# simeonjunker/retr

Measured on AMD Instinct MI355X. Metric: RefCOCO images/sec (train fwd+bwd) at 1/2/4/8 GPUs; greedy-decode refs/sec, higher is better.
Workload: dtype bf16; 1 GPU; cfg2: ResNet-50 + 6-enc/6-dec d_model 256, 640x640, batch 16/GPU, fwd+CE+bwd+allreduce+clip+AdamW; global_batch=16, seq_len=128, parallelism=dp1

## Files before the change

### retr_amd/csrc/conv.hip

```cpp
#include <algorithm>
#include <cstring>
#include <vector>

#include "gemm2.hpp"
#include "panel.hpp"
#include "epilogues.hpp"
#include "../../include/retr_hip.h"

using namespace retr;

namespace retr {
bool conv3x3_direct_ok(int H, int W, int CI, int CO);
int conv3x3_fwd_direct(const bf16* x, const bf16* w, const float* bias, bf16* y, int relu, int Nb,
                       int H, int W, int CI, int CO, hipStream_t st);
int conv3x3_dgrad_direct(const bf16* dy, const bf16* wt, bf16* dx, const bf16* addend,
                         const bf16* gate, int Nb, int H, int W, int CI_out, int CO_in,
                         hipStream_t st);
}

namespace {

struct Geom {
  int Nb, H, W, C, Co, KH, KW, s, p, d, OH, OW;
};

struct TapCur {
  int k, c, kw, khd, kwd;
};
RETR_DEVICE TapCur tap_cur(int k, int Cc, int KW, int dil) {
  TapCur t;
  t.k = k;
  int khw = k / Cc;
  t.c = k - khw * Cc;
  int kh = khw / KW;
  t.kw = khw - kh * KW;
  t.khd = kh * dil;
  t.kwd = t.kw * dil;
  return t;
}
RETR_DEVICE void tap_advance(TapCur& t, int d, int Cc, int KW, int dil) {
  t.k += d;
  t.c += d;
  while (t.c >= Cc) {
    t.c -= Cc;
    if (++t.kw == KW) {
      t.kw = 0;
      t.kwd = 0;
      t.khd += dil;
    } else {
      t.kwd += dil;
    }
  }
}

template <typename T>
struct ConvFwdA {
  static constexpr bool kContig = true;
  const T* x;
  Geom g;
  int M, K;
  struct Ctx { const T* img; int ihb, iwb; bool ok; };
  using KCur = TapCur;
  RETR_DEVICE Ctx row_ctx(int r) const {
    Ctx c;
    c.ok = r < M;
    int rr = c.ok ? r : 0;
    int hw = g.OH * g.OW;
    int n = rr / hw, rem = rr - n * hw;
    int oh = rem / g.OW, ow = rem - oh * g.OW;
    c.img = x + (long)n * g.H * g.W * g.C;
    c.ihb = oh * g.s - g.p;
    c.iwb = ow * g.s - g.p;
    return c;
  }
  RETR_DEVICE KCur kcur(int k) const { return tap_cur(k, g.C, g.KW, g.d); }
  RETR_DEVICE void advance(KCur& t, int d) const { tap_advance(t, d, g.C, g.KW, g.d); }
  RETR_DEVICE const void* addr(const Ctx& c, const KCur& t) const {
    if (!c.ok || t.k >= K) return nullptr;
    int ih = c.ihb + t.khd, iw = c.iwb + t.kwd;
    if ((unsigned)ih >= (unsigned)g.H || (unsigned)iw >= (unsigned)g.W) return nullptr;
    return c.img + ((long)ih * g.W + iw) * g.C + t.c;
  }
};

template <typename T>
struct ConvFwdAU {
  static constexpr bool kContig = true;
  static constexpr bool kUniformK = true;
  const T* x;
  Geom g;
  int M, K;
  struct Ctx { const T* base; unsigned mask; };
  struct KCur { int c0, t, kh, kw, off; };
  RETR_DEVICE Ctx row_ctx_c(int r, int coff) const {
    Ctx c;
    const bool ok = r < M;
    const int rr = ok ? r : 0;
    const int hw = g.OH * g.OW;
    const int n = rr / hw, rem = rr - n * hw;
    const int oh = rem / g.OW, ow = rem - oh * g.OW;
    const int ihb = oh * g.s - g.p, iwb = ow * g.s - g.p;
    c.base = x + (((long)n * g.H + ihb) * g.W + iwb) * g.C + coff;
    unsigned m = 0;
    if (ok) {
      for (int kh = 0; kh < g.KH; ++kh)
        for (int kw = 0; kw < g.KW; ++kw)
          if ((unsigned)(ihb + kh * g.d) < (unsigned)g.H &&
              (unsigned)(iwb + kw * g.d) < (unsigned)g.W)
            m |= 1u << (kh * g.KW + kw);
    }
    c.mask = m;
    return c;
  }
  RETR_DEVICE Ctx row_ctx(int r) const { return row_ctx_c(r, 0); }
  RETR_DEVICE void set_off(KCur& t) const { t.off = (t.kh * g.d * g.W + t.kw * g.d) * g.C + t.c0; }
  RETR_DEVICE KCur kcur(int k) const {
    KCur t;
    t.t = k / g.C;
    t.c0 = k - t.t * g.C;
    t.kh = t.t / g.KW;
    t.kw = t.t - t.kh * g.KW;
    set_off(t);
    return t;
  }
  RETR_DEVICE void advance(KCur& t, int d) const {
    t.c0 += d;
    if (t.c0 >= g.C) {
      t.c0 -= g.C;
      ++t.t;
      if (++t.kw == g.KW) {
        t.kw = 0;
        ++t.kh;
      }
    }
    set_off(t);
  }
  RETR_DEVICE const void* addr(const Ctx& c, const KCur& t) const {
    if (!((c.mask >> t.t) & 1u)) return nullptr;
    return c.base + t.off;
  }
  RETR_DEVICE const void* addr_or(const Ctx& c, const KCur& t, const void* fb) const {
    return ((c.mask >> t.t) & 1u) ? (const void*)(c.base + t.off) : fb;
  }
};

template <typename T>
struct ConvDgradA {
  static constexpr bool kContig = true;
  const T* gr;
  Geom g;
  int M, K;
  struct Ctx { const T* img; int ihp, iwp; bool ok; };
  using KCur = TapCur;
  RETR_DEVICE Ctx row_ctx(int r) const {
    Ctx c;
    c.ok = r < M;
    int rr = c.ok ? r : 0;
    int hw = g.H * g.W;
    int n = rr / hw, rem = rr - n * hw;
    int ih = rem / g.W, iw = rem - ih * g.W;
    c.img = gr + (long)n * g.OH * g.OW * g.Co;
    c.ihp = ih + g.p;
    c.iwp = iw + g.p;
    return c;
  }
  RETR_DEVICE KCur kcur(int k) const { return tap_cur(k, g.Co, g.KW, g.d); }
  RETR_DEVICE void advance(KCur& t, int d) const { tap_advance(t, d, g.Co, g.KW, g.d); }
  RETR_DEVICE const void* addr(const Ctx& c, const KCur& t) const {
    if (!c.ok || t.k >= K) return nullptr;
    int th = c.ihp - t.khd, tw = c.iwp - t.kwd;
    if (th < 0 || tw < 0) return nullptr;
    int oh = th, ow = tw;
    if (g.s != 1) {
      oh = th / g.s;
      ow = tw / g.s;
      if (oh * g.s != th || ow * g.s != tw) return nullptr;
    }
    if (oh >= g.OH || ow >= g.OW) return nullptr;
    return c.img + ((long)oh * g.OW + ow) * g.Co + t.c;
  }
};

template <typename T>
struct ConvDgradAU {
  static constexpr bool kContig = true;
  static constexpr bool kUniformK = true;
  const T* gr;
  Geom g;
  int M, K;
  struct Ctx { const T* base; unsigned mask; };
  struct KCur { int c0, t, kh, kw, off; };
  RETR_DEVICE Ctx row_ctx_c(int r, int coff) const {
    Ctx c;
    const bool ok = r < M;
    const int rr = ok ? r : 0;
    const int hw = g.H * g.W;
    const int n = rr / hw, rem = rr - n * hw;
    const int ih = rem / g.W, iw = rem - ih * g.W;
    const int ihp = ih + g.p, iwp = iw + g.p;
    c.base = gr + (((long)n * g.OH + ihp) * g.OW + iwp) * g.Co + coff;
    unsigned m = 0;
    if (ok) {
      for (int kh = 0; kh < g.KH; ++kh)
        for (int kw = 0; kw < g.KW; ++kw)
          if ((unsigned)(ihp - kh * g.d) < (unsigned)g.OH &&
              (unsigned)(iwp - kw * g.d) < (unsigned)g.OW)
            m |= 1u << (kh * g.KW + kw);
    }
    c.mask = m;
    return c;
  }
  RETR_DEVICE Ctx row_ctx(int r) const { return row_ctx_c(r, 0); }
  RETR_DEVICE void set_off(KCur& t) const {
    t.off = t.c0 - (t.kh * g.d * g.OW + t.kw * g.d) * g.Co;
  }
  RETR_DEVICE KCur kcur(int k) const {
    KCur t;
    t.t = k / g.Co;
    t.c0 = k - t.t * g.Co;
    t.kh = t.t / g.KW;
    t.kw = t.t - t.kh * g.KW;
    set_off(t);
    return t;
  }
  RETR_DEVICE void advance(KCur& t, int d) const {
    t.c0 += d;
    if (t.c0 >= g.Co) {
      t.c0 -= g.Co;
      ++t.t;
      if (++t.kw == g.KW) {
        t.kw = 0;
        ++t.kh;
      }
    }
    set_off(t);
  }
  RETR_DEVICE const void* addr(const Ctx& c, const KCur& t) const {
    if (!((c.mask >> t.t) & 1u)) return nullptr;
    return c.base + t.off;
  }
  RETR_DEVICE const void* addr_or(const Ctx& c, const KCur& t, const void* fb) const {
    return ((c.mask >> t.t) & 1u) ? (const void*)(c.base + t.off) : fb;
  }
};

template <typename T>
struct ConvWgradB {
  static constexpr bool kContig = false;
  const T* x;
  Geom g;
  int rows, M;
  int adv_q, adv_r;
  struct Ctx { int khd, kwd; long off; bool ok; };
  struct KCur { int m, oh, ow; long base; };
  RETR_DEVICE Ctx row_ctx(int r) const {
    Ctx c;
    c.ok = r < rows;
    int rr = c.ok ? r : 0;
    int khw = rr / g.C;
    const int ci = rr - khw * g.C;
    int kh = khw / g.KW, kw = khw - kh * g.KW;
    c.khd = kh * g.d - g.p;
    c.kwd = kw * g.d - g.p;
    c.off = ((long)c.khd * g.W + c.kwd) * g.C + ci;
    return c;
  }
  RETR_DEVICE KCur kcur(int m) const {
    KCur k;
    k.m = m;
    int hw = g.OH * g.OW;
    const int n = m / hw;
    int rem = m - n * hw;
    k.oh = rem / g.OW;
    k.ow = rem - k.oh * g.OW;
    k.base = (((long)n * g.H + k.oh * g.s) * g.W + k.ow * g.s) * g.C;
    return k;
  }
  RETR_DEVICE void advance(KCur& k, int d) const {
    k.m += d;
    if (d != Elem<T>::BK) {
      k = kcur(k.m);
      return;
    }
    const long rowC = (long)g.s * g.W * g.C;
    k.ow += adv_r;
    k.oh += adv_q;
    k.base += (long)adv_q * rowC + (long)adv_r * g.s * g.C;
    if (k.ow >= g.OW) {
      k.ow -= g.OW;
      k.oh += 1;
      k.base += rowC - (long)g.OW * g.s * g.C;
    }
    while (k.oh >= g.OH) {
      k.oh -= g.OH;
      k.base += ((long)g.H - (long)g.OH * g.s) * g.W * g.C;
    }
  }
  RETR_DEVICE const void* addr(const Ctx& c, const KCur& k) const {
    if (!c.ok || k.m >= M) return nullptr;
    int ih = k.oh * g.s + c.khd, iw = k.ow * g.s + c.kwd;
    if ((unsigned)ih >= (unsigned)g.H || (unsigned)iw >= (unsigned)g.W) return nullptr;
    return x + k.base + c.off;
  }
};

template <typename T>
struct ConvWgradB32 {
  static constexpr bool kContig = false;
  const T* x;
  Geom g;
  int rows, M;
  int adv_q, adv_r;
  int d_step, d_row, d_img;
  struct Ctx { int khd, kwd, off; bool ok; };
  struct KCur { int m, oh, ow, base; };
  RETR_DEVICE Ctx row_ctx(int r) const {
    Ctx c;
    c.ok = r < rows;
    const int rr = c.ok ? r : 0;
    const int khw = rr / g.C;
// ... 131 lines not shown
    c.mask = m;
    return c;
  }
  RETR_DEVICE Ctx row_ctx(int r) const { return row_ctx_c(r, 0); }
  RETR_DEVICE void set_off(KCur& t) const { t.off = t.c0 - (t.ti * g.OW + t.tj) * g.Co; }
  RETR_DEVICE KCur kcur(int k) const {
    KCur t;
    t.t = k / g.Co;
    t.c0 = k - t.t * g.Co;
    t.ti = t.t / ph.nkw;
    t.tj = t.t - t.ti * ph.nkw;
    set_off(t);
    return t;
  }
  RETR_DEVICE void advance(KCur& t, int d) const {
    t.c0 += d;
    if (t.c0 >= g.Co) {
      t.c0 -= g.Co;
      ++t.t;
      if (++t.tj == ph.nkw) {
        t.tj = 0;
        ++t.ti;
      }
    }
    set_off(t);
  }
  RETR_DEVICE const void* addr(const Ctx& c, const KCur& t) const {
    if (!((c.mask >> t.t) & 1u)) return nullptr;
    return c.base + t.off;
  }
  RETR_DEVICE const void* addr_or(const Ctx& c, const KCur& t, const void* fb) const {
    return ((c.mask >> t.t) & 1u) ? (const void*)(c.base + t.off) : fb;
  }
};

template <typename T>
struct DgradPhaseWU {
  static constexpr bool kContig = true;
  static constexpr bool kUniformK = true;
  const T* wt;
  Geom g;
  Phase ph;
  int rows, K;
  struct Ctx { const T* row; int klim; };
  struct KCur { int k, c0, ti, tj, off; };
  RETR_DEVICE Ctx row_ctx_c(int r, int coff) const {
    return Ctx{wt + (long)(r < rows ? r : 0) * g.KH * g.KW * g.Co + coff, r < rows ? K : 0};
  }
  RETR_DEVICE Ctx row_ctx(int r) const { return row_ctx_c(r, 0); }
  RETR_DEVICE void set_off(KCur& t) const {
    t.off = ((ph.a + 2 * t.ti) * g.KW + ph.b + 2 * t.tj) * g.Co + t.c0;
  }
  RETR_DEVICE KCur kcur(int k) const {
    KCur t;
    t.k = k;
    const int tap = k / g.Co;
    t.c0 = k - tap * g.Co;
    t.ti = tap / ph.nkw;
    t.tj = tap - t.ti * ph.nkw;
    set_off(t);
    return t;
  }
  RETR_DEVICE void advance(KCur& t, int d) const {
    t.k += d;
    t.c0 += d;
    if (t.c0 >= g.Co) {
      t.c0 -= g.Co;
      if (++t.tj == ph.nkw) {
        t.tj = 0;
        ++t.ti;
      }
    }
    set_off(t);
  }
  RETR_DEVICE const void* addr(const Ctx& c, const KCur& t) const {
    return t.k < c.klim ? (const void*)(c.row + t.off) : nullptr;
  }
  RETR_DEVICE const void* addr_or(const Ctx& c, const KCur& t, const void* fb) const {
    return t.k < c.klim ? (const void*)(c.row + t.off) : fb;
  }
};

template <typename T>
struct DgradPhaseW {
  static constexpr bool kContig = true;
  const T* wt;
  Geom g;
  Phase ph;
  int rows, K;
  struct Ctx { const T* row; bool ok; };
  struct KCur { int k, c, ti, tj; };
  RETR_DEVICE Ctx row_ctx(int r) const {
    return Ctx{wt + (long)(r < rows ? r : 0) * g.KH * g.KW * g.Co, r < rows};
  }
  RETR_DEVICE KCur kcur(int k) const {
    KCur t;
    t.k = k;
    const int tap = k / g.Co;
    t.c = k - tap * g.Co;
    t.ti = tap / ph.nkw;
    t.tj = tap - t.ti * ph.nkw;
    return t;
  }
  RETR_DEVICE void advance(KCur& t, int d) const {
    t.k += d;
    t.c += d;
    while (t.c >= g.Co) {
      t.c -= g.Co;
      if (++t.tj == ph.nkw) {
        t.tj = 0;
        ++t.ti;
      }
    }
  }
  RETR_DEVICE const void* addr(const Ctx& c, const KCur& t) const {
    if (!c.ok || t.k >= K) return nullptr;
    const int kh = ph.a + 2 * t.ti, kw = ph.b + 2 * t.tj;
    return c.row + ((long)kh * g.KW + kw) * g.Co + t.c;
  }
};

template <class EP>
struct EpiPhaseRows {
  EP ep;
  int Hp, Wp, H, W, ih0, iw0;
  static constexpr bool kRowSum = false;
  float* rowsum = nullptr;
  RETR_DEVICE int map(int m) const {
    const int hw = Hp * Wp;
    const int n = m / hw, rem = m - n * hw;
    const int i = rem / Wp, j = rem - i * Wp;
    return (n * H + ih0 + 2 * i) * W + iw0 + 2 * j;
  }
  RETR_DEVICE void apply(int m, int n, float v) const { ep.apply(map(m), n, v); }
  RETR_DEVICE void apply8(int m, int n, float (&v)[8]) const { ep.apply8(map(m), n, v); }
  using Pre = typename EP::Pre;
  RETR_DEVICE void fetch8(int m, int n, Pre& p) const { ep.fetch8(map(m), n, p); }
  RETR_DEVICE void apply8p(int m, int n, float (&v)[8], const Pre& p) const {
    ep.apply8p(map(m), n, v, p);
  }
  RETR_DEVICE void empty_split(int, int) const {}
  RETR_DEVICE bool lane_contiguous() const { return false; }
};

inline bool prefer_tile64(int M, int N, int K, bool dense1x1, bool res_small_k) {
  if (retr_tune_get(RETR_TUNE_BIG_TILE) != 0) return false;
  if (res_small_k) return true;
  if (M <= 8192 && (N <= 512 || K <= 512)) return true;
  return dense1x1 && N >= 1024 && K <= 512 && M <= 32768;
}

template <int FAM, typename T, class LA, class LB, class EP>
int launch_auto(const LA& la, const LB& lb, const EP& ep, int M, int N, int K, int splits,
                hipStream_t st, const char* what, bool dense1x1 = false,
                bool res_small_k = false) {
  if constexpr (sizeof(T) == 2) {
    return launch_big<FAM>(la, lb, ep, M, N, K, splits, st, what,
                           prefer_tile64(M, N, K, dense1x1, res_small_k));
  } else {
    if (N >= 128 && M >= 4096) return launch_gemm<FAM, T, 128, 128>(la, lb, ep, M, N, K, splits, st, what);
    return launch_gemm<FAM, T, 64, 64>(la, lb, ep, M, N, K, splits, st, what);
  }
}

struct WgradPlan {
  int tile;
  int splits;
};

template <typename T>
WgradPlan wgrad_plan(int R, int Ncols, int Mp, bool dense1x1) {
  constexpr int BK = Elem<T>::BK;
  WgradPlan p{64, 1};
  if (R >= 128 && Ncols >= 128) p.tile = sizeof(T) == 2 ? 128 : 129;
  const int tt = retr_tune_get(RETR_TUNE_CONV_WGRAD_TILE);
  if (sizeof(T) == 2 && R >= 64 && Ncols >= 64 &&
      (tt == 1 || (tt == 0 && dense1x1 && (R <= 128 || Ncols <= 128 || Mp <= 8192))))
    p.tile = 65;
  if (p.tile == 65 && tt == 3) p.tile = 66;
  const int bm = (p.tile == 64 || p.tile == 65 || p.tile == 66) ? 64 : 128;
  const int bn = bm;
  const long tiles = (long)cdiv(R, bm) * cdiv(Ncols, bn);
  const int ksteps = cdiv(Mp, BK);
  const int tune = retr_tune_get(RETR_TUNE_CONV_WGRAD_SPLITS);
  long smax = ksteps / 8;
  if (smax > 128) smax = 128;
  if (smax < 1) smax = 1;
  long s;
  if (tune >= 2) {
    s = tune < smax ? tune : smax;
  } else if (tune == 1 || (p.tile != 128 && p.tile != 65 && p.tile != 66)) {
    s = (512 + tiles - 1) / tiles;
    if (s > smax) s = smax;
  } else {
    const long slots = p.tile == 66 ? 2048 : p.tile == 65 ? 1024 : 512;
    const double slab_cost = p.tile == 128 ? 0.016 : 0.004;
    s = 1;
    double best = 1e30;
    for (long c = 1; c <= smax; ++c) {
      const long kc = cdiv(ksteps, (int)c);
      const long rounds = (tiles * cdiv(ksteps, (int)kc) + slots - 1) / slots;
      const double cost = (double)rounds * (kc + 2) + slab_cost * (double)tiles * c;
      if (cost < best) { best = cost; s = c; }
    }
  }
  if (s < 1) s = 1;
  const int kchunk = cdiv(ksteps, (int)s) * BK;
  p.splits = cdiv(Mp, kchunk);
  return p;
}

template <int FAM, typename T, class LA, class LB>
int launch_wgrad(const LA& la, const LB& lb, float* ws, long ldws, int R, int Ncols, int Mp,
                 hipStream_t st, const char* what, bool dense1x1) {
  const WgradPlan p = wgrad_plan<T>(R, Ncols, Mp, dense1x1);
  const int s = p.splits;
  EpiAccF32 ep{ws, ldws, 0, 0, 1, nullptr};
  ep.split_stride = s > 1 ? (long)R * ldws : 0;
  ep.set_vec();
  if constexpr (sizeof(T) == 2) {
    if (p.tile == 128 && !dense1x1)
      return launch_gemm2<FAM, 128, 128, 4, 2, 2>(la, lb, ep, R, Ncols, Mp, s, st, what);
    if (p.tile == 128) return launch_gemm2<FAM, 128, 128, 2, 2, 2>(la, lb, ep, R, Ncols, Mp, s, st, what);
    if (p.tile == 65) return launch_gemm2<FAM, 64, 64, 2, 2, 2>(la, lb, ep, R, Ncols, Mp, s, st, what);
    if (p.tile == 66) return launch_gemm2<FAM, 64, 64, 2, 2, 1>(la, lb, ep, R, Ncols, Mp, s, st, what);
  } else {
    if (p.tile == 129) return launch_gemm<FAM, T, 128, 128>(la, lb, ep, R, Ncols, Mp, s, st, what);
  }
  return launch_gemm<FAM, T, 64, 64>(la, lb, ep, R, Ncols, Mp, s, st, what);
}

template <typename T>
int conv_fwd_t(const void* x, Geom g, const void* w, const float* bias, const void* res, void* y,
               int relu, hipStream_t st) {
  int M = g.Nb * g.OH * g.OW, N = g.Co, K = g.KH * g.KW * g.C;
  DenseK<T> lb{(const T*)w, (long)K, N, K};
  EpiFwd<T, T> ep{(T*)y, (long)N, bias, (const T*)res, (long)N, relu ? 2 : 0, DropoutParams{0, 0, 1.f}, 0};
  ep.set_vec();
  if (g.KH == 1 && g.KW == 1 && g.s == 1 && g.p == 0) {
    DenseK<T> la{(const T*)x, (long)g.C, M, K};
    if constexpr (sizeof(T) == 2) {
      if (K <= 256 && K % 64 == 0 && N >= 1024 && retr_tune_get(RETR_TUNE_PANEL) == 1 &&
          retr_tune_get(RETR_TUNE_PANEL_CONV) == 1)
        return launch_panel<kFamConvFwd>(la, lb, ep, M, N, K, st, "conv_fwd_1x1");
    }
    return launch_auto<kFamConvFwd, T>(la, lb, ep, M, N, K, 1, st, "conv_fwd_1x1", true,
                                       res != nullptr && K <= 64);
  }
  if constexpr (sizeof(T) == 2) {
    if (g.KH == 3 && g.KW == 3 && g.s == 1 && g.p == 1 && g.d == 1 && !res && relu &&
        conv3x3_direct_ok(g.H, g.W, g.C, g.Co))
      return conv3x3_fwd_direct((const bf16*)x, (const bf16*)w, bias, (bf16*)y, relu, g.Nb, g.H,
                                g.W, g.C, g.Co, st);
  }
  if (sizeof(T) == 2 && g.C % 64 == 0 && g.KH * g.KW > 1 && g.KH * g.KW <= 32) {
    ConvFwdAU<T> la{(const T*)x, g, M, K};
    return launch_auto<kFamConvFwd, T>(la, lb, ep, M, N, K, 1, st, "conv_fwd");
  }
  ConvFwdA<T> la{(const T*)x, g, M, K};
  return launch_auto<kFamConvFwd, T>(la, lb, ep, M, N, K, 1, st, "conv_fwd");
}

__global__ void dgrad_phase_fill_kernel(bf16* dx, const bf16* addend, const bf16* gate, int H,
                                        int W, int C, long chunks, int zmask) {
  const long i = blockIdx.x * (long)blockDim.x + threadIdx.x;
  if (i >= chunks) return;
  const int cpp = C / 8;
  const long p = i / cpp;
  const int c = (int)(i - p * cpp) * 8;
  const int iw = (int)(p % W), ih = (int)((p / W) % H);
  if (!((zmask >> ((ih & 1) * 2 + (iw & 1))) & 1)) return;
  const long off = p * C + c;
  bf16x8 v;
  if (addend) {
    v = *(const bf16x8*)(addend + off);
  } else {
#pragma unroll
    for (int e = 0; e < 8; ++e) v[e] = (bf16)0.f;
  }
  if (gate) {
    const bf16x8 gg = *(const bf16x8*)(gate + off);
#pragma unroll
    for (int e = 0; e < 8; ++e)
      if (!((float)gg[e] > 0.f)) v[e] = (bf16)0.f;
  }
  *(bf16x8*)(dx + off) = v;
}

template <typename T>
int conv_dgrad_t(const void* dy, Geom g, const void* wt, void* dx, const void* addend,
                 const void* gate, hipStream_t st) {
  int M = g.Nb * g.H * g.W, N = g.C, K = g.KH * g.KW * g.Co;
  DenseK<T> lb{(const T*)wt, (long)K, N, K};
  EpiDgrad<T, T, T> ep{(T*)dx, (long)N, (const T*)addend, (long)N, (const T*)gate, (long)N};
  ep.set_vec();
  if (g.KH == 1 && g.KW == 1 && g.s == 1 && g.p == 0) {
    DenseK<T> la{(const T*)dy, (long)g.Co, M, K};
    if constexpr (sizeof(T) == 2) {
      if (K <= 256 && K % 64 == 0 && N >= 1024 && retr_tune_get(RETR_TUNE_PANEL) == 1 &&
          retr_tune_get(RETR_TUNE_PANEL_CONV) == 1)
        return launch_panel<kFamConvDgrad>(la, lb, ep, M, N, K, st, "conv_dgrad_1x1");
    }
    return launch_auto<kFamConvDgrad, T>(la, lb, ep, M, N, K, 1, st, "conv_dgrad_1x1", true);
  }
  if (g.s == 2 && g.d == 1) {
    int zmask = 0;
    for (int a = 0; a < 2; ++a)
      for (int bb = 0; bb < 2; ++bb) {
        const int nkh = g.KH > a ? (g.KH - a + 1) / 2 : 0;
        const int nkw = g.KW > bb ? (g.KW - bb + 1) / 2 : 0;
        if (nkh * nkw == 0) {
          const int ih0 = ((a - g.p) % 2 + 2) % 2, iw0 = ((bb - g.p) % 2 + 2) % 2;
          zmask |= 1 << (ih0 * 2 + iw0);
        }
      }
    const bool inplace = addend != nullptr && addend == dx;
    if (zmask && (inplace || (sizeof(T) == 2 && N % 8 == 0))) {
      if (!inplace) {
        const long chunks = (long)M * (N / 8);
        hipLaunchKernelGGL(dgrad_phase_fill_kernel, dim3((unsigned)cdiv(chunks, 256)), dim3(256),
                           0, st, (bf16*)dx, (const bf16*)addend, (const bf16*)gate, g.H, g.W, N,
                           chunks, zmask);
        if (int e = retr_check_launch("conv_dgrad_phase_fill")) return e;
      }
    } else {
      zmask = 0;
    }
    for (int a = 0; a < 2; ++a)
      for (int bb = 0; bb < 2; ++bb) {
        Phase ph;
        ph.a = a;
        ph.b = bb;
        ph.ih0 = ((a - g.p) % 2 + 2) % 2;
        ph.iw0 = ((bb - g.p) % 2 + 2) % 2;
        ph.Hp = g.H > ph.ih0 ? (g.H - ph.ih0 + 1) / 2 : 0;
        ph.Wp = g.W > ph.iw0 ? (g.W - ph.iw0 + 1) / 2 : 0;
        ph.nkh = g.KH > a ? (g.KH - a + 1) / 2 : 0;
        ph.nkw = g.KW > bb ? (g.KW - bb + 1) / 2 : 0;
        const int Mp = g.Nb * ph.Hp * ph.Wp, Kp = ph.nkh * ph.nkw * g.Co;
        if (Mp == 0) continue;
        if (Kp == 0 && (zmask >> (ph.ih0 * 2 + ph.iw0) & 1)) continue;
        EpiPhaseRows<EpiDgrad<T, T, T>> pe{ep, ph.Hp, ph.Wp, g.H, g.W, ph.ih0, ph.iw0};
        if (sizeof(T) == 2 && g.Co % 64 == 0 && ph.nkh * ph.nkw <= 32) {
          ConvDgradPhaseAU<T> pa{(const T*)dy, g, ph, Mp, Kp};
          DgradPhaseWU<T> pb{(const T*)wt, g, ph, N, Kp};
          if constexpr (sizeof(T) == 2) {
            if (N <= 128 && Mp >= 65536 && retr_tune_get(RETR_TUNE_BIG_TILE) == 0 &&
                retr_tune_get(RETR_TUNE_SHORTK) != 1) {
              if (int e = launch_gemm2<kFamConvDgrad, 64, 128, 2, 2, 1>(pa, pb, pe, Mp, N, Kp, 1,
                                                                          st, "conv_dgrad_s2"))
                return e;
              continue;
            }
          }
          if (int e = launch_auto<kFamConvDgrad, T>(pa, pb, pe, Mp, N, Kp, 1, st, "conv_dgrad_s2"))
            return e;
          continue;
        }
        ConvDgradPhaseA<T> pa{(const T*)dy, g, ph, Mp, Kp};
        DgradPhaseW<T> pb{(const T*)wt, g, ph, N, Kp};
        if (int e = launch_auto<kFamConvDgrad, T>(pa, pb, pe, Mp, N, Kp, 1, st, "conv_dgrad_s2"))
          return e;
      }
    return 0;
  }
  if constexpr (sizeof(T) == 2) {
    if (g.KH == 3 && g.KW == 3 && g.s == 1 && g.p == 1 && g.d == 1 &&
        conv3x3_direct_ok(g.H, g.W, g.Co, g.C))
      return conv3x3_dgrad_direct((const bf16*)dy, (const bf16*)wt, (bf16*)dx,
                                  (const bf16*)addend, (const bf16*)gate, g.Nb, g.H, g.W, g.Co,
                                  g.C, st);
  }
  if (sizeof(T) == 2 && g.s == 1 && g.Co % 64 == 0 && g.KH * g.KW <= 32) {
    ConvDgradAU<T> la{(const T*)dy, g, M, K};
    return launch_auto<kFamConvDgrad, T>(la, lb, ep, M, N, K, 1, st, "conv_dgrad");
  }
  ConvDgradA<T> la{(const T*)dy, g, M, K};
  return launch_auto<kFamConvDgrad, T>(la, lb, ep, M, N, K, 1, st, "conv_dgrad");
}

template <typename T>
int conv_wgrad_t(const void* dy, const void* x, Geom g, float* ws, hipStream_t st) {
  int Mp = g.Nb * g.OH * g.OW;
  int R = g.Co, Ncols = g.KH * g.KW * g.C;
  DenseT<T> la{(const T*)dy, (long)g.Co, R, Mp};
  if (g.KH == 1 && g.KW == 1 && g.s == 1 && g.p == 0) {
    DenseT<T> lb{(const T*)x, (long)g.C, Ncols, Mp};
    return launch_wgrad<kFamConvWgrad, T>(la, lb, ws, (long)Ncols, R, Ncols, Mp, st, "conv_wgrad_1x1",
                                          true);
  }
  constexpr int BK = Elem<T>::BK;
  if constexpr (sizeof(T) == 2) {
    if ((long)g.Nb * g.H * g.W * g.C < (1L << 31) && g.OH * g.OW >= BK &&
        retr_tune_get(RETR_TUNE_WGRAD_B32) != 1) {
      const int q = BK / g.OW, r = BK % g.OW;
      ConvWgradB32<T> lb{(const T*)x, g, Ncols, Mp, q, r,
                         (q * g.s * g.W + r * g.s) * g.C,
                         g.s * g.W * g.C - g.OW * g.s * g.C,
                         (g.H - g.OH * g.s) * g.W * g.C};
      return launch_wgrad<kFamConvWgrad, T>(la, lb, ws, (long)Ncols, R, Ncols, Mp, st,
                                            "conv_wgrad", false);
    }
  }
  ConvWgradB<T> lb{(const T*)x, g, Ncols, Mp, BK / g.OW, BK % g.OW};
  return launch_wgrad<kFamConvWgrad, T>(la, lb, ws, (long)Ncols, R, Ncols, Mp, st, "conv_wgrad", false);
}

template <typename T>
__global__ void conv_pack_kernel(const float* w, const float* bnw, const float* bnb,
                                 const float* bnrm, const float* bnrv, const float* conv_bias,
                                 int Co, int Ci, int KH, int KW, int Cp, T* wout, T* wtout,
                                 float* bias_out, float* scale_out) {
  long total = (long)Co * KH * KW * Cp;
  for (long i = blockIdx.x * (long)blockDim.x + threadIdx.x; i < total;
       i += (long)gridDim.x * blockDim.x) {
    int ci = i % Cp;
    long t = i / Cp;
    int kw = t % KW;
    t /= KW;
    int kh = t % KH;
    int co = (int)(t / KH);
    float scale = 1.f;
    if (bnw) scale = bnw[co] * (1.0f / sqrtf(bnrv[co] + 1e-5f));
    float v = ci < Ci ? w[(((long)co * Ci + ci) * KH + kh) * KW + kw] * scale : 0.f;
    wout[i] = from_f<T>(v);
    if (wtout) wtout[(((long)ci * KH + kh) * KW + kw) * Co + co] = from_f<T>(v);
    if (ci == 0 && kh == 0 && kw == 0) {
      float b;
      if (bnw) b = bnb[co] - bnrm[co] * scale;
      else b = conv_bias ? conv_bias[co] : 0.f;
      if (bias_out) bias_out[co] = b;
      if (scale_out) scale_out[co] = scale;
    }
  }
}

__global__ void wgrad_unpack4_kernel(const float* ws, const float* scale, float* grad, int Co,
                                     int Ci, int Cp, int KHW, int accumulate, int splits) {
  const int c4 = Ci / 4;
  const long total = (long)Co * KHW * c4;
  const long slab = (long)Co * KHW * Cp;
  for (long i = blockIdx.x * (long)blockDim.x + threadIdx.x; i < total;
       i += (long)gridDim.x * blockDim.x) {
    const int ci = (int)(i % c4) * 4;
    const long t = i / c4;
    const int tap = (int)(t % KHW), co = (int)(t / KHW);
    const float* src = ws + ((long)co * KHW + tap) * Cp + ci;
    f32x4 v = *(const f32x4*)src;
    int s = 1;
    for (; s + 7 < splits; s += 8) {
      f32x4 u[8];
#pragma unroll
      for (int k = 0; k < 8; ++k) u[k] = *(const f32x4*)(src + (s + k) * slab);
#pragma unroll
      for (int k = 0; k < 8; ++k) v += u[k];
    }
    for (; s < splits; ++s) v += *(const f32x4*)(src + s * slab);
    const float sc = scale ? scale[co] : 1.f;
    float* dst = grad + ((long)co * Ci + ci) * KHW + tap;
#pragma unroll
    for (int e = 0; e < 4; ++e) {
      const float x = v[e] * sc;
      dst[(long)e * KHW] = accumulate ? dst[(long)e * KHW] + x : x;
    }
  }
}

template <int NW>
__global__ void __launch_bounds__(NW * 64)
wgrad_unpack4w_kernel(const float* ws, const float* scale, float* grad, int Co, int Ci, int Cp,
                      int KHW, int accumulate, int splits) {
  __shared__ f32x4 red[NW][64];
  const int lane = threadIdx.x & 63, w = threadIdx.x >> 6;
  const int c4 = Ci / 4;
  const long total = (long)Co * KHW * c4;
  const long slab = (long)Co * KHW * Cp;
  const long i = (long)blockIdx.x * 64 + lane;
  int ci = 0, tap = 0, co = 0;
  f32x4 v = {0.f, 0.f, 0.f, 0.f};
  if (i < total) {
    ci = (int)(i % c4) * 4;
    const long t = i / c4;
    tap = (int)(t % KHW);
    co = (int)(t / KHW);
    const float* src = ws + ((long)co * KHW + tap) * Cp + ci;
    int s = w;
    for (; s + 7 * NW < splits; s += 8 * NW) {
      f32x4 u[8];
#pragma unroll
      for (int k = 0; k < 8; ++k) u[k] = *(const f32x4*)(src + (long)(s + k * NW) * slab);
#pragma unroll
      for (int k = 0; k < 8; ++k) v += u[k];
    }
    for (; s < splits; s += NW) v += *(const f32x4*)(src + (long)s * slab);
  }
  if constexpr (NW > 1) {
    red[w][lane] = v;
    __syncthreads();
    if (w != 0) return;
#pragma unroll
    for (int k = 1; k < NW; ++k) v += red[k][lane];
  }
  if (i >= total) return;
  const float sc = scale ? scale[co] : 1.f;
  float* dst = grad + ((long)co * Ci + ci) * KHW + tap;
#pragma unroll
  for (int e = 0; e < 4; ++e) {
    const float x = v[e] * sc;
    dst[(long)e * KHW] = accumulate ? dst[(long)e * KHW] + x : x;
  }
}

__global__ void wgrad_unpack_kernel(const float* ws, const float* scale, float* grad, int Co,
                                    int Ci, int Cp, int KH, int KW, int accumulate, int splits) {
  const long total = (long)Co * Ci * KH * KW;
  const long slab = (long)Co * KH * KW * Cp;
  for (long i = blockIdx.x * (long)blockDim.x + threadIdx.x; i < total;
       i += (long)gridDim.x * blockDim.x) {
    int kw = i % KW;
    long t = i / KW;
    int kh = t % KH;
    t /= KH;
    int ci = t % Ci;
    int co = (int)(t / Ci);
    const long src = ((long)co * KH * KW + kh * KW + kw) * Cp + ci;
    float v = ws[src];
    int s = 1;
    for (; s + 7 < splits; s += 8) {
      float t[8];
#pragma unroll
      for (int u = 0; u < 8; ++u) t[u] = ws[src + (s + u) * slab];
#pragma unroll
      for (int u = 0; u < 8; ++u) v += t[u];
    }
    for (; s < splits; ++s) v += ws[src + s * slab];
    if (scale) v *= scale[co];
    grad[i] = accumulate ? grad[i] + v : v;
  }
}

constexpr int kPackGroup = 16;
constexpr int kPackPerThread = 4;

struct PackGroup {
  retr_conv_pack_desc d[kPackGroup];
  int blk0[kPackGroup + 1];
  int n;
};

template <typename T>
__global__ void __launch_bounds__(256) conv_pack_group_kernel(PackGroup g) {
  const int bid = blockIdx.x;
  int p = 0;
#pragma unroll
  for (int i = 1; i < kPackGroup; ++i)
    if (i < g.n && bid >= g.blk0[i]) p = i;
  const retr_conv_pack_desc& d = g.d[p];
  const int Co = d.Co, Ci = d.Ci, KH = d.KH, KW = d.KW, Cp = d.Cp;
  const long total = (long)Co * KH * KW * Cp;
  const long base = ((long)(bid - g.blk0[p]) * 256 + threadIdx.x) * kPackPerThread;
  const float* bnw = d.bn_w;
#pragma unroll
  for (int u = 0; u < kPackPerThread; ++u) {
    const long i = base + u;
    if (i >= total) break;
    const int ci = (int)(i % Cp);
    long t = i / Cp;
    const int kw = (int)(t % KW);
    t /= KW;
    const int kh = (int)(t % KH);
    const int co = (int)(t / KH);
    float scale = 1.f;
    if (bnw) scale = bnw[co] * (1.0f / sqrtf(d.bn_rv[co] + 1e-5f));
    const float v = ci < Ci ? d.w[(((long)co * Ci + ci) * KH + kh) * KW + kw] * scale : 0.f;
    ((T*)d.w_out)[i] = from_f<T>(v);
    if (d.wt_out) ((T*)d.wt_out)[(((long)ci * KH + kh) * KW + kw) * Co + co] = from_f<T>(v);
    if (ci == 0 && kh == 0 && kw == 0) {
      float b;
      if (bnw) b = d.bn_b[co] - d.bn_rm[co] * scale;
      else b = d.conv_bias ? d.conv_bias[co] : 0.f;
      if (d.bias_out) d.bias_out[co] = b;
      if (d.scale_out) d.scale_out[co] = scale;
    }
  }
}

template <typename T, int KHW>
__global__ void __launch_bounds__(256) conv_pack_tiled_group_kernel(PackGroup g) {
  extern __shared__ __attribute__((aligned(16))) char smem[];
  T* tile = (T*)smem;
  __shared__ float sc[64];
  const int bid = blockIdx.x;
  int p = 0;
#pragma unroll
  for (int i = 1; i < kPackGroup; ++i)
    if (i < g.n && bid >= g.blk0[i]) p = i;
  const retr_conv_pack_desc& d = g.d[p];
  const int Co = d.Co, Cp = d.Cp;
  const int t = bid - g.blk0[p], tn = Cp / 64;
  const int co0 = (t / tn) * 64, ci0 = (t % tn) * 64;
  const int tid = threadIdx.x;
  if (tid < 64) {
    const int co = co0 + tid;
    float scale = 1.f;
    if (d.bn_w) scale = d.bn_w[co] * (1.0f / sqrtf(d.bn_rv[co] + 1e-5f));
    sc[tid] = scale;
// ... 693 lines not shown
```

### retr_amd/csrc/conv3x3.hip

```cpp
#include <cstring>

#include "gemm2.hpp"
#include "epilogues.hpp"
#include "../../include/retr_hip.h"

using namespace retr;

namespace {

template <bool FLIP>
struct TapW {
  static constexpr bool kContig = true;
  static constexpr bool kUniformK = true;
  const bf16* p;
  int rows, CP;
  struct Ctx { const bf16* row; bool ok; };
  struct KCur { int t, c64, off; };
  RETR_DEVICE Ctx row_ctx_c(int r, int coff) const {
    return Ctx{p + (long)(r < rows ? r : 0) * 9 * CP + coff, r < rows};
  }
  RETR_DEVICE Ctx row_ctx(int r) const { return row_ctx_c(r, 0); }
  RETR_DEVICE KCur kcur(int) const { return KCur{0, 0, (FLIP ? 8 : 0) * CP}; }
  RETR_DEVICE void advance(KCur& k, int) const {
    if (++k.t == 9) {
      k.t = 0;
      k.c64 += 64;
    }
    k.off = (FLIP ? 8 - k.t : k.t) * CP + k.c64;
  }
  RETR_DEVICE const void* addr_or(const Ctx& c, const KCur& k, const void* fb) const {
    return c.ok ? (const void*)(c.row + k.off) : fb;
  }
  RETR_DEVICE const void* addr(const Ctx& c, const KCur& k) const {
    return c.ok ? (const void*)(c.row + k.off) : nullptr;
  }
};

template <int TH, int TW, int BN, int RB, int S>
constexpr size_t c3_main_lds() {
  return ((size_t)(TH + 2) * (TW + 2) * RB + 255) / 256 * 256 + (size_t)S * BN * kBKBytes;
}
template <int TH, int TW, int BN, int WM, int RB, int S>
constexpr int epi_passes() {
  int p = 1;
  while (p < WM && (size_t)TH * TW * (BN + 4) * 4 / p > c3_main_lds<TH, TW, BN, RB, S>()) p *= 2;
  return p;
}

template <int TH, int TW, int BN, int WM, int WN, int RB, int S, bool DGRAD, class EP>
__global__ void __launch_bounds__(WM * WN * 64, 2)
conv3x3_kernel(const bf16* __restrict__ x, const bf16* __restrict__ w, EP ep, int H, int W,
               int CI, int CO, int tiles_x, int tiles_y, int tiles_n) {
  constexpr int NT = WM * WN * 64;
  constexpr int BM = TH * TW;
  constexpr int HH = TH + 2, HW = TW + 2, HP = HH * HW;
  constexpr int WTM = BM / WM, WTN = BN / WN;
  constexpr int TM = WTM / 16, TN = WTN / 16;
  static_assert(WTM % 16 == 0 && WTN % 16 == 0, "wave tile");
  constexpr int HALO_BYTES = (HP * RB + 255) / 256 * 256;
  static_assert(RB % 16 == 0 && RB >= 128, "halo row");
  constexpr int WST = BN * kBKBytes;
  static_assert(S == 2 || S == 3, "weight ring");
  constexpr int HCH = (HP * 8 + NT - 1) / NT;
  using LB = TapW<DGRAD>;
  using SB = GStager<BN, NT, LB>;
  constexpr int LPT = SB::NCH;
  extern __shared__ __attribute__((aligned(16))) char smem[];
  char* halo = smem;
  char* wst = smem + HALO_BYTES;

  const int tid = threadIdx.x, lane = tid & 63;
  const int wave = __builtin_amdgcn_readfirstlane(tid >> 6);
  const int wm = wave / WN, wn = wave % WN;
  const int nblk = gridDim.x;
  const int bid = xcd_remap(blockIdx.x, nblk);
  const int tpi = tiles_x * tiles_y;
  const int nt = bid % tiles_n;
  const int rest = bid / tiles_n;
  const int img = rest / tpi, tt = rest % tpi;
  const int y0 = (tt / tiles_x) * TH, x0 = (tt % tiles_x) * TW;
  const int n0 = nt * BN;
  const int nchunks = CI / 64;
  const int nsteps = nchunks * 9;

  const bf16* xin = x + (long)img * H * W * CI;
  auto halo_load = [&](int c, u32x4 (&r)[HCH]) {
#pragma unroll
    for (int i = 0; i < HCH; ++i) {
      const int q = tid + NT * i;
      const int hp = q >> 3, j = q & 7;
      const int gy = y0 + hp / HW - 1, gx = x0 + hp % HW - 1;
      const bool ok = q < HP * 8 && (unsigned)gy < (unsigned)H && (unsigned)gx < (unsigned)W;
      const bf16* src = ok ? xin + ((long)gy * W + gx) * CI + c * 64 + j * 8
                           : (const bf16*)g_zero_page;
      r[i] = *(const u32x4*)src;
    }
  };
  auto halo_store = [&](const u32x4 (&r)[HCH]) {
#pragma unroll
    for (int i = 0; i < HCH; ++i) {
      const int q = tid + NT * i;
      if (q < HP * 8) *(u32x4*)(halo + (q >> 3) * RB + (q & 7) * 16) = r[i];
    }
  };

  int abase[TM];
#pragma unroll
  for (int i = 0; i < TM; ++i) {
    const int p = wm * WTM + 16 * i + (lane & 15);
    abase[i] = ((p / TW) * HW + p % TW) * RB + (lane >> 4) * 16;
  }

  SB sb;
  const LB lb{w, CO, CI};
  sb.init(lb, n0, tid, 0);

  f32x4 acc[TM][TN];
#pragma unroll
  for (int i = 0; i < TM; ++i)
#pragma unroll
    for (int j = 0; j < TN; ++j) acc[i][j] = f32x4{0.f, 0.f, 0.f, 0.f};

  u32x4 hr[HCH];
  halo_load(0, hr);
  sb.issue(lb, wst, wave);
  if (S == 3 && nsteps > 1) sb.issue(lb, wst + WST, wave);
  halo_store(hr);

  int s = 0;
  for (int c = 0; c < nchunks; ++c) {
    if (c > 0) {
      raw_barrier();
      halo_store(hr);
    }
    const bool more = c + 1 < nchunks;
#pragma unroll
    for (int t = 0; t < 9; ++t, ++s) {
      const bool nx = S == 3 && s + 1 < nsteps;
      const bool hh = more && (t == 1 || (S == 3 && t == 2));
      if (nx && hh) wait_vmcnt_lgkm0<LPT + HCH>();
      else if (nx) wait_vmcnt_lgkm0<LPT>();
      else if (hh) wait_vmcnt_lgkm0<HCH>();
      else wait_vmcnt_lgkm0<0>();
      raw_barrier();
      if (s + S - 1 < nsteps) sb.issue(lb, wst + ((s + S - 1) % S) * WST, wave);
      if (t == 0 && more) halo_load(c + 1, hr);
      const char* B = wst + (s % S) * WST;
      const int tapoff = ((t / 3) * HW + t % 3) * RB;
#pragma unroll
      for (int ks = 0; ks < 2; ++ks) {
        u32x4 af[TM], bfr[TN];
#pragma unroll
        for (int i = 0; i < TM; ++i) af[i] = *(const u32x4*)(halo + abase[i] + tapoff + ks * 64);
#pragma unroll
        for (int j = 0; j < TN; ++j)
          bfr[j] = Stager<bf16, BN, LB>::frag(B, wn * WTN + 16 * j, ks, lane);
#pragma unroll
        for (int i = 0; i < TM; ++i)
#pragma unroll
          for (int j = 0; j < TN; ++j) mfma_step<bf16>(acc[i][j], af[i], bfr[j]);
      }
    }
  }
  (void)LPT;
  __syncthreads();

  constexpr int CS = BN + 4;
  constexpr int EPB = epi_passes<TH, TW, BN, WM, RB, S>();
  constexpr int BAND = BM / EPB;
  constexpr int CH = BN / 8;
  float* ct = (float*)smem;
#pragma unroll
  for (int pass = 0; pass < EPB; ++pass) {
    if (pass > 0) __syncthreads();
    if (wm / (WM / EPB) == pass) {
#pragma unroll
      for (int i = 0; i < TM; ++i)
#pragma unroll
        for (int j = 0; j < TN; ++j)
#pragma unroll
          for (int e = 0; e < 4; ++e)
            ct[(wm * WTM - pass * BAND + 16 * i + 4 * (lane >> 4) + e) * CS + wn * WTN + 16 * j +
               (lane & 15)] = acc[i][j][e];
    }
    __syncthreads();
    for (int q = tid; q < BAND * CH; q += NT) {
      const int mb = q / CH, cc = (q % CH) * 8;
      const int m = pass * BAND + mb;
      const int y = y0 + m / TW, xx = x0 + m % TW;
      if (y >= H || xx >= W || n0 + cc >= CO) continue;
      const int row = (img * H + y) * W + xx;
      const f32x4 lo = *(const f32x4*)(ct + mb * CS + cc);
      const f32x4 hi = *(const f32x4*)(ct + mb * CS + cc + 4);
      float v[8] = {lo[0], lo[1], lo[2], lo[3], hi[0], hi[1], hi[2], hi[3]};
      ep.apply8(row, n0 + cc, v);
    }
  }
}

template <int TH, int TW, int BN, int WM, int WN, int RB, int S>
constexpr size_t c3_lds() {
  constexpr size_t main = c3_main_lds<TH, TW, BN, RB, S>();
  constexpr size_t epi = (size_t)TH * TW * (BN + 4) * 4 / epi_passes<TH, TW, BN, WM, RB, S>();
  return main > epi ? main : epi;
}

template <int TH, int TW, int BN, int WM, int WN, int RB, bool DGRAD, int S = 2, class EP>
int launch_c3(const bf16* x, const bf16* w, const EP& ep, int Nb, int H, int W, int CI, int CO,
              hipStream_t st, const char* what) {
  const int tiles_x = cdiv(W, TW), tiles_y = cdiv(H, TH), tiles_n = cdiv(CO, BN);
  const long blocks = (long)Nb * tiles_x * tiles_y * tiles_n;
  constexpr size_t lds = c3_lds<TH, TW, BN, WM, WN, RB, S>();
  auto kern = conv3x3_kernel<TH, TW, BN, WM, WN, RB, S, DGRAD, EP>;
  if constexpr (lds > 65536) {
    static bool attr_set = false;
    if (!attr_set) {
      (void)hipFuncSetAttribute((const void*)kern, hipFuncAttributeMaxDynamicSharedMemorySize,
                                (int)lds);
      attr_set = true;
    }
  }
  hipLaunchKernelGGL(kern, dim3((unsigned)blocks), dim3(WM * WN * 64), lds, st, x, w, ep, H, W,
                     CI, CO, tiles_x, tiles_y, tiles_n);
  return retr_check_launch(what);
}

template <bool DGRAD, class EP>
int run_c3(const bf16* x, const bf16* w, const EP& ep, int Nb, int H, int W, int CI, int CO,
           hipStream_t st, const char* what) {
  switch (retr_tune_get(RETR_TUNE_C3_TILE)) {
    case 1: return launch_c3<8, 16, 128, 4, 2, 160, DGRAD>(x, w, ep, Nb, H, W, CI, CO, st, what);
    case 2: return launch_c3<8, 20, 128, 2, 4, 160, DGRAD>(x, w, ep, Nb, H, W, CI, CO, st, what);
    case 3: return launch_c3<4, 16, 128, 2, 4, 160, DGRAD>(x, w, ep, Nb, H, W, CI, CO, st, what);
    case 4: return launch_c3<8, 16, 64, 4, 2, 160, DGRAD>(x, w, ep, Nb, H, W, CI, CO, st, what);
    case 5: return launch_c3<16, 16, 128, 4, 2, 160, DGRAD>(x, w, ep, Nb, H, W, CI, CO, st, what);
    case 6:
      if (CO % 256 == 0) return launch_c3<8, 20, 256, 2, 4, 160, DGRAD>(x, w, ep, Nb, H, W, CI, CO, st, what);
      break;
    case 7: return launch_c3<4, 20, 128, 1, 4, 160, DGRAD>(x, w, ep, Nb, H, W, CI, CO, st, what);
    case 8: return launch_c3<8, 16, 128, 2, 2, 160, DGRAD>(x, w, ep, Nb, H, W, CI, CO, st, what);
    case 9: return launch_c3<4, 20, 128, 1, 4, 144, DGRAD>(x, w, ep, Nb, H, W, CI, CO, st, what);
    case 10: return launch_c3<8, 16, 128, 4, 2, 144, DGRAD>(x, w, ep, Nb, H, W, CI, CO, st, what);
    case 11: return launch_c3<8, 20, 128, 2, 4, 144, DGRAD>(x, w, ep, Nb, H, W, CI, CO, st, what);
    case 12: return launch_c3<8, 16, 128, 4, 2, 160, DGRAD, 3>(x, w, ep, Nb, H, W, CI, CO, st, what);
    case 13: return launch_c3<8, 20, 128, 2, 4, 160, DGRAD, 3>(x, w, ep, Nb, H, W, CI, CO, st, what);
    default: break;
  }
  if (W == 20) return launch_c3<8, 20, 128, 2, 4, 160, DGRAD>(x, w, ep, Nb, H, W, CI, CO, st, what);
  return launch_c3<8, 16, 128, 4, 2, 160, DGRAD>(x, w, ep, Nb, H, W, CI, CO, st, what);
}

}

namespace retr {

bool conv3x3_direct_ok(int H, int W, int CI, int CO) {
  const int mode = retr_tune_get(RETR_TUNE_CONV3X3);
  if (mode == 1) return false;
  if (mode == 2) return CI % 64 == 0 && CO % 128 == 0 && H >= 8 && W >= 16;
  return CI % 64 == 0 && CO % 128 == 0 && H >= 8 && (W >= 32 || W == 20);
}

int conv3x3_fwd_direct(const bf16* x, const bf16* w, const float* bias, bf16* y, int relu, int Nb,
                       int H, int W, int CI, int CO, hipStream_t st) {
  EpiFwd<bf16, bf16> ep{y, (long)CO, bias, (const bf16*)nullptr, (long)CO, relu ? 2 : 0,
                        DropoutParams{0, 0, 1.f}, 0};
  ep.set_vec();
  return run_c3<false>(x, w, ep, Nb, H, W, CI, CO, st, "conv3x3_fwd");
}

int conv3x3_dgrad_direct(const bf16* dy, const bf16* wt, bf16* dx, const bf16* addend,
                         const bf16* gate, int Nb, int H, int W, int CI_out, int CO_in,
                         hipStream_t st) {
  EpiDgrad<bf16, bf16, bf16> ep{dx, (long)CO_in, addend, (long)CO_in, gate, (long)CO_in};
  ep.set_vec();
  return run_c3<true>(dy, wt, ep, Nb, H, W, CI_out, CO_in, st, "conv3x3_dgrad");
}

}
```

Before: 1724 images/s.

## Add direct implicit-GEMM kernel for stride-2 3x3 conv data gradient

Adds a stride-2 variant of the direct 3x3 conv kernel for the data gradient. It splits the output into four parity phases, each with its own accumulator set, so every tap hits exactly one phase. A 1-pixel halo over the gradient is staged in shared memory, and the phase results are written back interleaved through the epilogue. This replaces the generic phase-decomposed GEMM path (zero fill plus separate launches) for ResNet stride-2 3x3 backward. The cost is four times the accumulator registers, which can drop occupancy to one block per CU, and new index logic that has to be correct.

```diff
diff --git a/retr_amd/csrc/conv.hip b/retr_amd/csrc/conv.hip
--- a/retr_amd/csrc/conv.hip
+++ b/retr_amd/csrc/conv.hip
@@ -16,6 +16,10 @@
 int conv3x3_dgrad_direct(const bf16* dy, const bf16* wt, bf16* dx, const bf16* addend,
                          const bf16* gate, int Nb, int H, int W, int CI_out, int CO_in,
                          hipStream_t st);
+bool conv3x3_s2_dgrad_ok(int Nb, int H, int W, int Co, int C);
+int conv3x3_s2_dgrad_direct(const bf16* dy, const bf16* wt, bf16* dx, const bf16* addend,
+                            const bf16* gate, int Nb, int H, int W, int Co, int C,
+                            hipStream_t st);
 }
 
 namespace {
@@ -753,6 +757,13 @@
         return launch_panel<kFamConvDgrad>(la, lb, ep, M, N, K, st, "conv_dgrad_1x1");
     }
     return launch_auto<kFamConvDgrad, T>(la, lb, ep, M, N, K, 1, st, "conv_dgrad_1x1", true);
+  }
+  if constexpr (sizeof(T) == 2) {
+    if (g.KH == 3 && g.KW == 3 && g.s == 2 && g.p == 1 && g.d == 1 &&
+        conv3x3_s2_dgrad_ok(g.Nb, g.H, g.W, g.Co, g.C))
+      return conv3x3_s2_dgrad_direct((const bf16*)dy, (const bf16*)wt, (bf16*)dx,
+                                     (const bf16*)addend, (const bf16*)gate, g.Nb, g.H, g.W, g.Co,
+                                     g.C, st);
   }
   if (g.s == 2 && g.d == 1) {
     int zmask = 0;
diff --git a/retr_amd/csrc/conv3x3.hip b/retr_amd/csrc/conv3x3.hip
--- a/retr_amd/csrc/conv3x3.hip
+++ b/retr_amd/csrc/conv3x3.hip
@@ -36,24 +36,36 @@
   }
 };
 
-template <int TH, int TW, int BN, int RB, int S>
+template <int TH, int TW, int BN, int RB, int S, int HX = 2>
 constexpr size_t c3_main_lds() {
-  return ((size_t)(TH + 2) * (TW + 2) * RB + 255) / 256 * 256 + (size_t)S * BN * kBKBytes;
-}
-template <int TH, int TW, int BN, int WM, int RB, int S>
+  return ((size_t)(TH + HX) * (TW + HX) * RB + 255) / 256 * 256 + (size_t)S * BN * kBKBytes;
+}
+template <int TH, int TW, int BN, int WM, int RB, int S, int HX = 2>
 constexpr int epi_passes() {
   int p = 1;
-  while (p < WM && (size_t)TH * TW * (BN + 4) * 4 / p > c3_main_lds<TH, TW, BN, RB, S>()) p *= 2;
+  while (p < WM && (size_t)TH * TW * (BN + 4) * 4 / p > c3_main_lds<TH, TW, BN, RB, S, HX>())
+    p *= 2;
   return p;
 }
 
-template <int TH, int TW, int BN, int WM, int WN, int RB, int S, bool DGRAD, class EP>
-__global__ void __launch_bounds__(WM * WN * 64, 2)
+template <int TH, int TW, int BN, int WM, int WN, int STRIDE>
+constexpr int c3_min_blocks() {
+  if (STRIDE == 1) return 2;
+  constexpr int acc = 4 * (TH * TW / WM / 16) * (BN / WN / 16) * 4;
+  return acc + 56 <= 1024 / (WM * WN) ? 2 : 1;
+}
+
+template <int TH, int TW, int BN, int WM, int WN, int RB, int S, bool DGRAD, int STRIDE, class EP>
+__global__ void __launch_bounds__(WM * WN * 64, (c3_min_blocks<TH, TW, BN, WM, WN, STRIDE>()))
 conv3x3_kernel(const bf16* __restrict__ x, const bf16* __restrict__ w, EP ep, int H, int W,
                int CI, int CO, int tiles_x, int tiles_y, int tiles_n) {
   constexpr int NT = WM * WN * 64;
   constexpr int BM = TH * TW;
-  constexpr int HH = TH + 2, HW = TW + 2, HP = HH * HW;
+  constexpr bool S2 = STRIDE == 2;
+  static_assert(STRIDE == 1 || (S2 && DGRAD), "stride 2: data gradient only");
+  constexpr int HX = S2 ? 1 : 2;
+  constexpr int NA = S2 ? 4 : 1;
+  constexpr int HH = TH + HX, HW = TW + HX, HP = HH * HW;
   constexpr int WTM = BM / WM, WTN = BN / WN;
   constexpr int TM = WTM / 16, TN = WTN / 16;
   static_assert(WTM % 16 == 0 && WTN % 16 == 0, "wave tile");
@@ -62,7 +74,7 @@
   constexpr int WST = BN * kBKBytes;
   static_assert(S == 2 || S == 3, "weight ring");
   constexpr int HCH = (HP * 8 + NT - 1) / NT;
-  using LB = TapW<DGRAD>;
+  using LB = TapW<DGRAD && !S2>;
   using SB = GStager<BN, NT, LB>;
   constexpr int LPT = SB::NCH;
   extern __shared__ __attribute__((aligned(16))) char smem[];
@@ -83,15 +95,16 @@
   const int nchunks = CI / 64;
   const int nsteps = nchunks * 9;
 
-  const bf16* xin = x + (long)img * H * W * CI;
+  const int IH = S2 ? (H - 1) / 2 + 1 : H, IW = S2 ? (W - 1) / 2 + 1 : W;
+  const bf16* xin = x + (long)img * IH * IW * CI;
   auto halo_load = [&](int c, u32x4 (&r)[HCH]) {
 #pragma unroll
     for (int i = 0; i < HCH; ++i) {
       const int q = tid + NT * i;
       const int hp = q >> 3, j = q & 7;
-      const int gy = y0 + hp / HW - 1, gx = x0 + hp % HW - 1;
-      const bool ok = q < HP * 8 && (unsigned)gy < (unsigned)H && (unsigned)gx < (unsigned)W;
-      const bf16* src = ok ? xin + ((long)gy * W + gx) * CI + c * 64 + j * 8
+      const int gy = y0 + hp / HW - (HX - 1), gx = x0 + hp % HW - (HX - 1);
+      const bool ok = q < HP * 8 && (unsigned)gy < (unsigned)IH && (unsigned)gx < (unsigned)IW;
+      const bf16* src = ok ? xin + ((long)gy * IW + gx) * CI + c * 64 + j * 8
                            : (const bf16*)g_zero_page;
       r[i] = *(const u32x4*)src;
     }
@@ -115,11 +128,13 @@
   const LB lb{w, CO, CI};
   sb.init(lb, n0, tid, 0);
 
-  f32x4 acc[TM][TN];
-#pragma unroll
-  for (int i = 0; i < TM; ++i)
-#pragma unroll
-    for (int j = 0; j < TN; ++j) acc[i][j] = f32x4{0.f, 0.f, 0.f, 0.f};
+  f32x4 acc[NA][TM][TN];
+#pragma unroll
+  for (int a = 0; a < NA; ++a)
+#pragma unroll
+    for (int i = 0; i < TM; ++i)
+#pragma unroll
+      for (int j = 0; j < TN; ++j) acc[a][i][j] = f32x4{0.f, 0.f, 0.f, 0.f};
 
   u32x4 hr[HCH];
   halo_load(0, hr);
@@ -146,7 +161,8 @@
       if (s + S - 1 < nsteps) sb.issue(lb, wst + ((s + S - 1) % S) * WST, wave);
       if (t == 0 && more) halo_load(c + 1, hr);
       const char* B = wst + (s % S) * WST;
-      const int tapoff = ((t / 3) * HW + t % 3) * RB;
+      const int tapoff = S2 ? ((t / 3 == 0) * HW + (t % 3 == 0)) * RB : ((t / 3) * HW + t % 3) * RB;
+      const int pa = S2 ? (t / 3 != 1) * 2 + (t % 3 != 1) : 0;
 #pragma unroll
       for (int ks = 0; ks < 2; ++ks) {
         u32x4 af[TM], bfr[TN];
@@ -158,7 +174,7 @@
 #pragma unroll
         for (int i = 0; i < TM; ++i)
 #pragma unroll
-          for (int j = 0; j < TN; ++j) mfma_step<bf16>(acc[i][j], af[i], bfr[j]);
+          for (int j = 0; j < TN; ++j) mfma_step<bf16>(acc[pa][i][j], af[i], bfr[j]);
       }
     }
   }
@@ -166,52 +182,58 @@
   __syncthreads();
 
   constexpr int CS = BN + 4;
-  constexpr int EPB = epi_passes<TH, TW, BN, WM, RB, S>();
+  constexpr int EPB = epi_passes<TH, TW, BN, WM, RB, S, HX>();
   constexpr int BAND = BM / EPB;
   constexpr int CH = BN / 8;
   float* ct = (float*)smem;
 #pragma unroll
-  for (int pass = 0; pass < EPB; ++pass) {
-    if (pass > 0) __syncthreads();
-    if (wm / (WM / EPB) == pass) {
-#pragma unroll
-      for (int i = 0; i < TM; ++i)
-#pragma unroll
-        for (int j = 0; j < TN; ++j)
-#pragma unroll
-          for (int e = 0; e < 4; ++e)
-            ct[(wm * WTM - pass * BAND + 16 * i + 4 * (lane >> 4) + e) * CS + wn * WTN + 16 * j +
-               (lane & 15)] = acc[i][j][e];
-    }
-    __syncthreads();
-    for (int q = tid; q < BAND * CH; q += NT) {
-      const int mb = q / CH, cc = (q % CH) * 8;
-      const int m = pass * BAND + mb;
-      const int y = y0 + m / TW, xx = x0 + m % TW;
-      if (y >= H || xx >= W || n0 + cc >= CO) continue;
-      const int row = (img * H + y) * W + xx;
-      const f32x4 lo = *(const f32x4*)(ct + mb * CS + cc);
-      const f32x4 hi = *(const f32x4*)(ct + mb * CS + cc + 4);
-      float v[8] = {lo[0], lo[1], lo[2], lo[3], hi[0], hi[1], hi[2], hi[3]};
-      ep.apply8(row, n0 + cc, v);
-    }
-  }
-}
-
-template <int TH, int TW, int BN, int WM, int WN, int RB, int S>
+  for (int a = 0; a < NA; ++a) {
+#pragma unroll
+    for (int pass = 0; pass < EPB; ++pass) {
+      if (a > 0 || pass > 0) __syncthreads();
+      if (wm / (WM / EPB) == pass) {
+#pragma unroll
+        for (int i = 0; i < TM; ++i)
+#pragma unroll
+          for (int j = 0; j < TN; ++j)
+#pragma unroll
+            for (int e = 0; e < 4; ++e)
+              ct[(wm * WTM - pass * BAND + 16 * i + 4 * (lane >> 4) + e) * CS + wn * WTN + 16 * j +
+                 (lane & 15)] = acc[a][i][j][e];
+      }
+      __syncthreads();
+      for (int q = tid; q < BAND * CH; q += NT) {
+        const int mb = q / CH, cc = (q % CH) * 8;
+        const int m = pass * BAND + mb;
+        const int y = S2 ? 2 * (y0 + m / TW) + (a >> 1) : y0 + m / TW;
+        const int xx = S2 ? 2 * (x0 + m % TW) + (a & 1) : x0 + m % TW;
+        if (y >= H || xx >= W || n0 + cc >= CO) continue;
+        const int row = (img * H + y) * W + xx;
+        const f32x4 lo = *(const f32x4*)(ct + mb * CS + cc);
+        const f32x4 hi = *(const f32x4*)(ct + mb * CS + cc + 4);
+        float v[8] = {lo[0], lo[1], lo[2], lo[3], hi[0], hi[1], hi[2], hi[3]};
+        ep.apply8(row, n0 + cc, v);
+      }
+    }
+  }
+}
+
+template <int TH, int TW, int BN, int WM, int WN, int RB, int S, int HX = 2>
 constexpr size_t c3_lds() {
-  constexpr size_t main = c3_main_lds<TH, TW, BN, RB, S>();
-  constexpr size_t epi = (size_t)TH * TW * (BN + 4) * 4 / epi_passes<TH, TW, BN, WM, RB, S>();
+  constexpr size_t main = c3_main_lds<TH, TW, BN, RB, S, HX>();
+  constexpr size_t epi = (size_t)TH * TW * (BN + 4) * 4 / epi_passes<TH, TW, BN, WM, RB, S, HX>();
   return main > epi ? main : epi;
 }
 
-template <int TH, int TW, int BN, int WM, int WN, int RB, bool DGRAD, int S = 2, class EP>
+template <int TH, int TW, int BN, int WM, int WN, int RB, bool DGRAD, int S = 2, int STRIDE = 1,
+          class EP>
 int launch_c3(const bf16* x, const bf16* w, const EP& ep, int Nb, int H, int W, int CI, int CO,
               hipStream_t st, const char* what) {
-  const int tiles_x = cdiv(W, TW), tiles_y = cdiv(H, TH), tiles_n = cdiv(CO, BN);
+  const int TWD = STRIDE == 2 ? (W - 1) / 2 + 1 : W, THD = STRIDE == 2 ? (H - 1) / 2 + 1 : H;
+  const int tiles_x = cdiv(TWD, TW), tiles_y = cdiv(THD, TH), tiles_n = cdiv(CO, BN);
   const long blocks = (long)Nb * tiles_x * tiles_y * tiles_n;
-  constexpr size_t lds = c3_lds<TH, TW, BN, WM, WN, RB, S>();
-  auto kern = conv3x3_kernel<TH, TW, BN, WM, WN, RB, S, DGRAD, EP>;
+  constexpr size_t lds = c3_lds<TH, TW, BN, WM, WN, RB, S, STRIDE == 2 ? 1 : 2>();
+  auto kern = conv3x3_kernel<TH, TW, BN, WM, WN, RB, S, DGRAD, STRIDE, EP>;
   if constexpr (lds > 65536) {
     static bool attr_set = false;
     if (!attr_set) {
@@ -250,12 +272,32 @@
   return launch_c3<8, 16, 128, 4, 2, 160, DGRAD>(x, w, ep, Nb, H, W, CI, CO, st, what);
 }
 
+template <class EP>
+int run_c3s2(const bf16* dy, const bf16* w, const EP& ep, int Nb, int H, int W, int CI, int CO,
+             hipStream_t st, const char* what) {
+  switch (retr_tune_get(RETR_TUNE_C3_TILE)) {
+    case 1: return launch_c3<8, 16, 128, 4, 2, 160, true, 2, 2>(dy, w, ep, Nb, H, W, CI, CO, st, what);
+    case 2: return launch_c3<8, 20, 128, 2, 4, 160, true, 2, 2>(dy, w, ep, Nb, H, W, CI, CO, st, what);
+    case 3: return launch_c3<8, 16, 64, 4, 2, 160, true, 2, 2>(dy, w, ep, Nb, H, W, CI, CO, st, what);
+    case 4: return launch_c3<8, 20, 64, 2, 4, 160, true, 2, 2>(dy, w, ep, Nb, H, W, CI, CO, st, what);
+    case 5: return launch_c3<4, 16, 128, 2, 4, 160, true, 2, 2>(dy, w, ep, Nb, H, W, CI, CO, st, what);
+    case 6: return launch_c3<4, 20, 64, 1, 4, 160, true, 2, 2>(dy, w, ep, Nb, H, W, CI, CO, st, what);
+    case 7: return launch_c3<8, 16, 128, 4, 2, 160, true, 3, 2>(dy, w, ep, Nb, H, W, CI, CO, st, what);
+    case 8: return launch_c3<8, 20, 128, 2, 4, 160, true, 3, 2>(dy, w, ep, Nb, H, W, CI, CO, st, what);
+    default: break;
+  }
+  const int OW = (W - 1) / 2 + 1;
+  if (OW % 20 == 0 && OW % 16 != 0)
+    return launch_c3<4, 20, 64, 1, 4, 160, true, 2, 2>(dy, w, ep, Nb, H, W, CI, CO, st, what);
+  return launch_c3<8, 16, 64, 4, 2, 160, true, 2, 2>(dy, w, ep, Nb, H, W, CI, CO, st, what);
+}
+
 }
 
 namespace retr {
 
 bool conv3x3_direct_ok(int H, int W, int CI, int CO) {
-  const int mode = retr_tune_get(RETR_TUNE_CONV3X3);
+  const int mode = retr_tune_get(RETR_TUNE_CONV3X3) & 3;
   if (mode == 1) return false;
   if (mode == 2) return CI % 64 == 0 && CO % 128 == 0 && H >= 8 && W >= 16;
   return CI % 64 == 0 && CO % 128 == 0 && H >= 8 && (W >= 32 || W == 20);
@@ -277,4 +319,21 @@
   return run_c3<true>(dy, wt, ep, Nb, H, W, CI_out, CO_in, st, "conv3x3_dgrad");
 }
 
-}
+bool conv3x3_s2_dgrad_ok(int Nb, int H, int W, int Co, int C) {
+  const int mode = retr_tune_get(RETR_TUNE_CONV3X3) >> 2;
+  const int OW = (W - 1) / 2 + 1;
+  (void)Nb;
+  if (mode == 1 || Co % 64 != 0 || C % 8 != 0 || OW < 16) return false;
+  if (mode == 2) return true;
+  return OW >= 20 && Co >= 128 && C >= 128 && C % 64 == 0;
+}
+
+int conv3x3_s2_dgrad_direct(const bf16* dy, const bf16* wt, bf16* dx, const bf16* addend,
+                            const bf16* gate, int Nb, int H, int W, int Co, int C,
+                            hipStream_t st) {
+  EpiDgrad<bf16, bf16, bf16> ep{dx, (long)C, addend, (long)C, gate, (long)C};
+  ep.set_vec();
+  return run_c3s2(dy, wt, ep, Nb, H, W, Co, C, st, "conv3x3_s2_dgrad");
+}
+
+}
```

Result: no change. 1735 images/s, median of 6 (+0.6%).
